# kcat/openal-soft

Measured on NVIDIA H100. Metric: voice-samples/s mixed (HRTF, bsinc24, 1024-frame updates), higher is better.
Workload: dtype f32

## Files before the change

### openal-soft_b200/csrc/mixer_kernels.cuh

```cuda
#pragma once
#include <cstddef>
#include <cstdint>
#include <cuda_runtime.h>

#include "voice_structs.hpp"
#include "async_ptx.cuh"

namespace b200mix {

constexpr int kLine = 1024;
constexpr int kHrirLen = 128;
constexpr int kHist = 64;
constexpr int kEdge = 24;
constexpr int kPad = 48;
constexpr int kResBuf = kLine + 256 + kPad;
constexpr int kSrcSizeMax = kResBuf - kEdge;
constexpr int kAccumLen = kLine + kHrirLen;
constexpr float kSilence = 0.00001f;
constexpr float kEps = 1.1920929e-07f;

constexpr uint32_t kVfStatic = 1u<<2, kVfLooping = 1u<<3, kVfHrtf = 1u<<4;
constexpr uint32_t kVfFading = 1u<<8, kVfHaveBuffer = 1u<<9, kVfCoefDirty = 1u<<10;
constexpr uint32_t kUpNoBuffer = 1u<<11;
constexpr uint32_t kVfChannelMask = 0xffu<<16;

struct alignas(16) BufferRec {
    const void *data;
    uint32_t frames, type, channels, pad;
};

struct alignas(16) VoiceRec {
    uint32_t state;
    uint32_t flags;
    uint32_t buffer, resampler;
    int32_t  pos; uint32_t frac, step, loop_start;
    uint32_t loop_end; float bsinc_sf; uint32_t bsinc_m, bsinc_l;
    uint32_t bsinc_off, tgt_delay0, tgt_delay1; float tgt_gain;
    uint32_t old_delay0, old_delay1; float old_gain; uint32_t send_mask;
    uint32_t send_slot[kMaxSends]; uint32_t pad2[2];
    float prev[kPad];
    float hist[kHist];
};

struct VoiceResult { int32_t position; uint32_t position_frac, flags, buffers_done; };

struct alignas(16) FilterRec {
    float cur[2][5]; float tgt[2][5];
    float z[2][2];
    int32_t counter[2];
    uint32_t active;
    uint32_t pad[5];
};
static_assert(sizeof(FilterRec) == 128, "FilterRec layout");

struct MixParams {
    VoiceRec *voices; const BufferRec *buffers;
    float2 *hrtf_tgt; float2 *hrtf_old;
    float *dry_cur; float *dry_tgt;
    float *partial;
    VoiceResult *results;
    const float *bsinc_tab[3];
    const float *cubic_tab[2];
    uint32_t max_voices, frames, ir_pad, cd, num_sends;
    float *xscratch;
    uint32_t *sendinfo;
    const uint32_t *order;
    uint32_t num_order;
    FilterRec *filt;
    uint32_t filt_paths;
    const float *dline;
    uint4 *qhdr; const uint32_t *queue;
    uint32_t *claim;
    const BufferRec *cbplan;
};

constexpr uint32_t kMaxQueue = 32, kNoLoop = 0xffffffffu;

constexpr uint32_t kSiSend = 1u, kSiPlaying = 2u, kSiDeferred = 4u, kSiDirty = 8u, kSiDry = 16u,
    kSiHrtf = 32u;

__device__ __forceinline__ void group_sync(int id, int count)
{
    if(id == 1) asm volatile("bar.sync 1, %0;" :: "r"(count) : "memory");
    else asm volatile("bar.sync 2, %0;" :: "r"(count) : "memory");
}

__device__ __forceinline__ bool group_sync_and(int id, int count, bool pred)
{
    uint32_t all;
    if(id == 1)
        asm volatile("{ .reg .pred p, q; setp.ne.u32 p, %1, 0; bar.red.and.pred q, 1, %2, p; selp.u32 %0, 1, 0, q; }"
            : "=r"(all) : "r"(uint32_t(pred)), "r"(count) : "memory");
    else
        asm volatile("{ .reg .pred p, q; setp.ne.u32 p, %1, 0; bar.red.and.pred q, 2, %2, p; selp.u32 %0, 1, 0, q; }"
            : "=r"(all) : "r"(uint32_t(pred)), "r"(count) : "memory");
    return all != 0u;
}

__device__ __forceinline__ bool exact16(float v)
{
    const float s = v*32768.0f;
    return s == rintf(s) && s >= -32768.0f && s <= 32767.0f;
}

__device__ __forceinline__ void prefetch_l2(const void *p)
{ asm volatile("prefetch.global.L2 [%0];" :: "l"(p)); }

__device__ __forceinline__ uint32_t sample_bytes(uint32_t type)
{ return type == 1u ? 2u : ((type == 0u || type >= 5u) ? 1u : (type == 4u ? 8u : 4u)); }

__device__ __forceinline__ void prefetch_span(const char *base, size_t bytes, size_t off,
    size_t len, int t, int gs)
{
    if(off >= bytes) return;
    if(off + len > bytes) len = bytes - off;
    const size_t first = off & ~size_t(127);
    for(size_t a = first + size_t(t)*128u;a < off + len;a += size_t(gs)*128u)
        prefetch_l2(base + a);
}

__device__ __forceinline__ float load_sample(const BufferRec &b, size_t idx)
{
    switch(b.type)
    {
    case 0: return (float(static_cast<const uint8_t*>(b.data)[idx]) - 128.0f) * (1.0f/128.0f);
    case 1: return float(static_cast<const int16_t*>(b.data)[idx]) * (1.0f/32768.0f);
    case 2: return float(static_cast<const int32_t*>(b.data)[idx]) * (1.0f/2147483648.0f);
    case 3: return static_cast<const float*>(b.data)[idx];
    case 4: return float(static_cast<const double*>(b.data)[idx]);
    }
    return 0.0f;
}

__device__ __forceinline__ void calc_buffer_size(uint32_t fracPos, uint32_t increment,
    uint32_t dstRemaining, uint32_t &dst, uint32_t &src)
{
    const uint32_t ext = increment <= 65536u;
    const uint64_t srcSize64 = ((uint64_t(dstRemaining - ext)*increment + fracPos) >> 16)
        + ext + kEdge;
    if(srcSize64 <= uint64_t(kSrcSizeMax)) { dst = dstRemaining; src = uint32_t(srcSize64); return; }
    const uint64_t dstSize64 = ((uint64_t(kSrcSizeMax - kEdge)<<16) - fracPos) / increment;
    if(dstSize64 < dstRemaining) { dst = uint32_t(dstSize64) & ~3u; src = kSrcSizeMax; return; }
    dst = dstRemaining; src = kSrcSizeMax;
}

__device__ __forceinline__ int32_t add_sat(int32_t a, int32_t b)
{
    long long r = (long long)a + b;
    r = r > 2147483647ll ? 2147483647ll : (r < -2147483648ll ? -2147483648ll : r);
    return int32_t(r);
}

__device__ __forceinline__ float to_float(uint8_t v) { return (float(v) - 128.0f) * (1.0f/128.0f); }
__device__ __forceinline__ float to_float(int16_t v) { return float(v) * (1.0f/32768.0f); }
__device__ __forceinline__ float to_float(int32_t v) { return float(v) * (1.0f/2147483648.0f); }
__device__ __forceinline__ float to_float(float v) { return v; }
__device__ __forceinline__ float to_float(double v) { return float(v); }
struct MulawByte { uint8_t v; };
struct AlawByte { uint8_t v; };
__device__ __forceinline__ float to_float(MulawByte b)
{
    const uint32_t u = (~uint32_t(b.v)) & 0xffu;
    const int s = int((((u & 0x0fu)<<3) + 0x84u) << ((u>>4)&7u)) - 0x84;
    return float((u & 0x80u) ? -s : s) * (1.0f/32768.0f);
}
__device__ __forceinline__ float to_float(AlawByte b)
{
    const uint32_t a = uint32_t(b.v) ^ 0x55u;
    const uint32_t e = (a>>4)&7u, m = a & 0x0fu;
    const int s = (e == 0u) ? int((m<<4) + 8u) : int(((m<<4) + 0x108u) << (e-1u));
    return float((a & 0x80u) ? s : -s) * (1.0f/32768.0f);
}

template<typename T> __device__ __forceinline__ T ld_raw(const T *p) { return __ldg(p); }
template<> __device__ __forceinline__ MulawByte ld_raw(const MulawByte *p)
{ return MulawByte{__ldg(reinterpret_cast<const uint8_t*>(p))}; }
template<> __device__ __forceinline__ AlawByte ld_raw(const AlawByte *p)
{ return AlawByte{__ldg(reinterpret_cast<const uint8_t*>(p))}; }

constexpr int kPackB = 688;
static_assert(kPackB >= (kResBuf + 8 + 1)/2 && kPackB + (kResBuf + 8 + 1)/2 <= kResBuf + 8 + 24
    && (kPackB % 32) == 16, "16-bit window copies must fit the float window's storage");

__device__ __forceinline__ float win_at(const float *win, bool packed, uint32_t k)
{
    if(!packed) return win[k];
    const uint16_t y = reinterpret_cast<const uint16_t*>(win)[k];
    return float(int(y) - 32768) * (1.0f/32768.0f);
}

struct FillArgs {
    float *dst; uint32_t count, uintPos, q0, firstRun, loopStart, loopSize, lastFrame, channels;
    bool looping, pastEnd, simpleWrap;
};

__device__ __forceinline__ void filter_clear(FilterRec &fr, int t)
{
    if(t < 10) fr.cur[t/5][t%5] = fr.tgt[t/5][t%5];
    else if(t < 14) fr.z[(t-10)>>1][(t-10)&1] = 0.0f;
    else if(t < 16) fr.counter[t-14] = 0;
}

template<typename T, int GS>
__device__ __forceinline__ void fill_window(const FillArgs &A, const T *__restrict__ src, int t)
{
    for(uint32_t k0 = t;k0 < A.count;k0 += 8u*GS)
    {
        T raw[8];
        #pragma unroll
        for(int u = 0;u < 8;++u)
        {
            uint32_t k = k0 + uint32_t(u)*GS;
            k = k < A.count ? k : A.count-1u;
            uint32_t q;
            if(!A.looping) q = min(A.uintPos + k, A.lastFrame);
            else if(k < A.firstRun) q = A.q0 + k;
            else if(A.simpleWrap) q = A.loopStart + (k - A.firstRun);
            else q = A.loopStart + (k - A.firstRun)%A.loopSize;
            raw[u] = ld_raw(src + size_t(q)*A.channels);
        }
        #pragma unroll
        for(int u = 0;u < 8;++u)
        {
            const uint32_t k = k0 + uint32_t(u)*GS;
            if(k < A.count) A.dst[k] = A.pastEnd ? 0.0f : to_float(raw[u]);
        }
    }
}

constexpr int kWinFloats = kResBuf + 8 + 24;
template<int CDR>
struct alignas(16) GroupSmem {
    static constexpr int kTabStride = kPad + 2;
    float win[kWinFloats];
    alignas(8) float tabF[32*kTabStride];
    alignas(8) float tabD[32*kTabStride];
    float x[CDR > 0 ? kLine : 1];
    float newGain[32];
    uint64_t tmaBar;
    uint32_t claimed;
};

struct alignas(16) FirStage {
    float x[kHist + kLine];
    float2 coefT[kHrirLen], coefO[kHrirLen];
};
static_assert(offsetof(VoiceRec, hist) % 16 == 0 && sizeof(VoiceRec) % 16 == 0,
    "VoiceRec::hist is a bulk-copy source: 16-byte aligned");

template<int GS, int OPT, int FP>
struct alignas(16) FirSmem {
    static constexpr int kLLen = FP + OPT*GS;
    static constexpr int kOLen = FP + kHist + FP + 32;
    float2 lLR[kLLen];
    float2 oLR[kOLen];
    FirStage st[2];
    uint64_t bar[2];
};

__device__ __forceinline__ float2 fma2_rn(float2 a, float2 b, float2 c)
{ return make_float2(__fmaf_rn(a.x, b.x, c.x), __fmaf_rn(a.y, b.y, c.y)); }

template<int OPT, int FP>
__device__ __forceinline__ void fir_pass(float2 (&acc)[OPT], const float2 *__restrict__ in,
    const float2 *__restrict__ coef, int irpad, int t0)
{
    constexpr int JB = 8;
    constexpr int W = OPT + JB - 1;
    for(int jb = 0;jb < irpad;jb += 2*JB)
    {
        const float2 *p = in + FP + t0 - jb - (JB-1);
        float2 w[W];
        #pragma unroll
        for(int k = 0;k < W;++k) w[k] = p[k];
        #pragma unroll
        for(int jj = 0;jj < JB;++jj)
        {
            const float2 c = coef[jb+jj];
            #pragma unroll
            for(int r = 0;r < OPT;++r)
                acc[r] = fma2_rn(c, w[r - jj + (JB-1)], acc[r]);
        }
        if(jb + JB >= irpad) break;
        #pragma unroll
        for(int k = W-1;k >= JB;--k) w[k] = w[k-JB];
        #pragma unroll
        for(int k = 0;k < JB;++k) w[k] = p[k - JB];
        #pragma unroll
        for(int jj = 0;jj < JB;++jj)
        {
            const float2 c = coef[jb+JB+jj];
            #pragma unroll
            for(int r = 0;r < OPT;++r)
                acc[r] = fma2_rn(c, w[r - jj + (JB-1)], acc[r]);
        }
    }
}

__device__ __forceinline__ uint32_t claim_voice(const MixParams &P, uint32_t &slot, int t, int bar,
    int gs, uint32_t groups)
{
    group_sync(bar, gs);
    if(t == 0)
    {
        uint32_t oi = atomicAdd(P.claim, 1u);
        if(oi >= P.num_order && atomicAdd(P.claim + 1, 1u) == groups - 1u)
        {
            atomicExch(P.claim, 0u);
            atomicExch(P.claim + 1, 0u);
        }
        slot = oi;
    }
    group_sync(bar, gs);
    return slot;
}


__device__ __forceinline__ bool voice_early_out(const MixParams &P, VoiceRec &rec, uint32_t v,
    uint32_t vstate, uint4 h1, int t)
{
    if(vstate != 1u && vstate != 2u)
    {
        if(t == 0)
        {
            if(P.results) P.results[v] = VoiceResult{int32_t(h1.x), h1.y, 1u<<7, 0u};
            if(P.sendinfo) P.sendinfo[v] = 0u;
        }
        return true;
    }
    if(h1.z < 1u)
    {
        if(t == 0)
        {
            if(vstate == 2u) rec.state = 0u;
            if(P.sendinfo) P.sendinfo[v] = 0u;
            if(P.results)
                P.results[v] = VoiceResult{int32_t(h1.x), h1.y, (vstate == 2u) ? (1u<<7) : 1u, 0u};
        }
        return true;
    }
    return false;
}

template<int GS>
__device__ __forceinline__ void build_phase_table(const MixParams &P, float *tabF, float *tabD,
    uint32_t resampler, uint32_t increment, uint4 h2, uint4 h3, int t,
    uint32_t &m, uint32_t &tapOff, uint32_t &ms)
{
    m = 0; tapOff = 0; ms = 5;
    if(resampler >= 4u)
    {
        m = h2.z;
        tapOff = kEdge - h2.w;
        const float *tab = P.bsinc_tab[(resampler-4u)>>1] + h3.x;
        const bool full = (increment > 65536u) && (resampler & 1u);
        const float sf = __uint_as_float(h2.y);
        const uint32_t rowLen = 2u*m;
        const float *tab2 = tab + 64u*m;
        ms = m + 1u;
        for(uint32_t c = t;c < rowLen;c += GS)
        {
            float *dstc = (c < m) ? (tabF + c) : (tabD + (c - m));
            #pragma unroll 1
            for(uint32_t p0 = 0;p0 < 32u;p0 += 8u)
            {
                float a[8], b[8];
                #pragma unroll
                for(int u = 0;u < 8;++u)
                {
                    a[u] = __ldg(tab + (p0+u)*rowLen + c);
                    b[u] = full ? __ldg(tab2 + (p0+u)*rowLen + c) : 0.0f;
                }
                #pragma unroll
                for(int u = 0;u < 8;++u)
                    dstc[(p0+u)*ms] = full ? fmaf(sf, b[u], a[u]) : a[u];
            }
        }
    }
    else if(resampler >= 2u)
    {
        m = 4; tapOff = kEdge - 1; ms = 5;
        const float *tab = P.cubic_tab[resampler-2u];
        for(uint32_t e = t;e < 128u;e += GS)
        {
            const uint32_t pi = e>>2, j = e&3u;
            tabF[pi*ms + j] = tab[pi*8u + j];
            tabD[pi*ms + j] = tab[pi*8u + 4u + j];
        }
    }
}

template<int GS>
__device__ __forceinline__ void prefetch_next_voices(const MixParams &P, uint32_t oi, uint32_t groups,
    int t)
{
    const uint32_t o2 = oi + 2u*groups, o1 = oi + groups;
    const uint32_t v2 = o2 < P.num_order ? P.order[o2] : 0xffffffffu;
    const uint32_t v1 = o1 < P.num_order ? P.order[o1] : 0xffffffffu;
    if(v2 < P.max_voices && t < 5)
        prefetch_l2(reinterpret_cast<const char*>(&P.voices[v2]) + t*128);
    if(v1 < P.max_voices)
    {
        const VoiceRec &nx = P.voices[v1];
        if((nx.state == 1u || nx.state == 2u) && (nx.flags & kVfHaveBuffer) && nx.step >= 1u)
        {
            const BufferRec nb = P.buffers[nx.buffer];
            const size_t fb = size_t(sample_bytes(nb.type))*nb.channels;
            const size_t bytes = size_t(nb.frames)*fb;
            const uint32_t p0 = nx.pos < 0 ? 0u : uint32_t(nx.pos);
            const size_t need = size_t((uint64_t(P.frames)*nx.step + nx.frac) >> 16) + kPad;
            const char *base = static_cast<const char*>(nb.data);
            prefetch_span(base, bytes, size_t(p0)*fb, need*fb, t, GS);
            if((nx.flags & kVfLooping) && p0 + need > nx.loop_end && nx.loop_end > p0)
                prefetch_span(base, bytes, size_t(nx.loop_start)*fb,
                    (p0 + need - nx.loop_end)*fb, t, GS);
        }
    }
}

template<int GS>
__device__ __forceinline__ void hold_end_sample(float *srcBuffer, uint32_t srcn, int t, int bar)
{
    const uint32_t avail = srcn < uint32_t(kEdge) ? srcn : uint32_t(kEdge);
    const uint32_t tofill = srcn > uint32_t(kEdge) ? srcn : uint32_t(kEdge);
    uint32_t best = 0;
    for(uint32_t i = 1;i < avail;++i)
        if(fabsf(srcBuffer[i]) < fabsf(srcBuffer[best])) best = i;
    const float held = srcBuffer[best];
    group_sync(bar, GS);
    for(uint32_t k = best+1+t;k < tofill;k += GS) srcBuffer[k] = held;
}

template<int GS>
__device__ __forceinline__ void pack_span16(float *win, const unsigned char *raw, uint32_t lead,
    uint32_t srcDelay, uint32_t count, int t, int bar)
{
    constexpr int NW = (kResBuf + 8 + 1)/2;
    constexpr int PER = (NW + GS - 1)/GS;
    static_assert((GS/32)*(32*PER - 1) >= NW + 1, "the warps' runs must cover every word");
    const uint32_t lane = uint32_t(t) & 31u;
    const uint32_t w0 = uint32_t(t >> 5)*(32u*PER - 1u) + lane;
    const uint32_t lo = uint32_t(kEdge) + srcDelay;
    const uint32_t nw = (min(lo + count + 8u, uint32_t(kResBuf + 8)) + 1u)/2u;
    const uint32_t off = lo - lead;
    const uint32_t *rw = reinterpret_cast<const uint32_t*>(raw) - int((off + 1u) >> 1);
    const uint32_t sh = (off & 1u)*16u;
    uint32_t wa[PER];
    #pragma unroll
    for(int u = 0;u < PER;++u)
    {
        const uint32_t w = w0 + uint32_t(u)*32u;
        wa[u] = (w <= nw && 2u*w + 1u >= lo) ? rw[w] : 0u;
    }
    #pragma unroll
    for(int u = 0;u < PER;++u)
    {
        const uint32_t w = w0 + uint32_t(u)*32u;
        uint32_t r1 = __shfl_sync(0xffffffffu, (u + 1 < PER && lane == 0u) ? wa[u + 1 < PER ? u + 1 : u] : wa[u],
            (lane + 1u) & 31u);
        if(u + 1 == PER && lane == 31u && w <= nw && 2u*w + 3u >= lo) r1 = rw[w + 1u];
        uint32_t a = __funnelshift_r(wa[u], r1, sh) ^ 0x80008000u;
        const int d = int(lo) - int(2u*w);
        const uint32_t m = (d >= 1 ? 0x0000ffffu : 0u) | (d >= 2 ? 0xffff0000u : 0u);
        a = (a & ~m) | (0x80008000u & m);
        if(u == 0 && w < uint32_t(kEdge/2))
            a = uint32_t(uint16_t(__float2int_rn(win[2u*w]*32768.0f) + 32768))
                | (uint32_t(uint16_t(__float2int_rn(win[2u*w + 1u]*32768.0f) + 32768)) << 16);
        wa[u] = a;
    }
    group_sync(bar, GS);
    uint32_t *pa = reinterpret_cast<uint32_t*>(win);
    uint32_t *pb = pa + kPackB;
    #pragma unroll
    for(int u = 0;u < PER;++u)
    {
        const uint32_t w = w0 + uint32_t(u)*32u;
        const uint32_t next = __shfl_sync(0xffffffffu, (u + 1 < PER && lane == 0u) ? wa[u + 1 < PER ? u + 1 : u] : wa[u],
            (lane + 1u) & 31u);
        if(w < nw)
        {
            if(u > 0 || lane > 0u || t < 32) pa[w] = wa[u];
            if(u + 1 < PER || lane < 31u) pb[w] = __funnelshift_r(wa[u], next, 16u);
        }
    }
}

template<int GS>
__device__ __forceinline__ bool stage_span_tma(float *win, uint64_t *tmaBar, uint32_t &tmaPhase,
    const BufferRec &buf, uint32_t flags, bool isQueue, bool looping, uint32_t loopStart,
    uint32_t loopEnd, uint32_t uintPos, uint32_t srcDelay, uint32_t count, bool pack, bool &packed,
    int t, int bar)
{
    if(isQueue || buf.type != 1u || buf.channels != 1u || ((flags >> 16) & 0xffu) != 0u || count == 0u)
        return false;
    const uint32_t loopSize = looping ? (loopEnd - loopStart) : 1u;
    const uint32_t q0 = !looping ? uintPos : ((uintPos < loopEnd) ? uintPos
        : ((uintPos-loopStart)%loopSize + loopStart));
    const uint32_t run1 = looping ? min(count, loopEnd - q0) : count;
    const uint32_t run2 = count - run1;
    const bool fits = looping ? (run2 <= loopSize && loopEnd <= buf.frames)
                              : (uintPos + count <= buf.frames);
    if(!fits) return false;
    const int16_t *base = static_cast<const int16_t*>(buf.data);
    const uintptr_t a1 = reinterpret_cast<uintptr_t>(base + q0);
    const uintptr_t a2 = reinterpret_cast<uintptr_t>(base + loopStart);
    const uint32_t lead1 = uint32_t(a1 & 15u) >> 1, lead2 = uint32_t(a2 & 15u) >> 1;
    const uint32_t bytes1 = ((run1 + lead1)*2u + 15u) & ~15u;
    const uint32_t bytes2 = run2 ? (((run2 + lead2)*2u + 15u) & ~15u) : 0u;
    constexpr uint32_t kWinBytes = uint32_t(kWinFloats*sizeof(float));
    unsigned char *wbytes = reinterpret_cast<unsigned char*>(win);
    unsigned char *raw2 = wbytes + kWinBytes - bytes2;
    unsigned char *raw1 = raw2 - bytes1;
    if(t == 0)
    {
        fence_proxy_async_smem();
        mbar_expect_tx(tmaBar, bytes1 + bytes2);
        bulk_g2s(raw1, reinterpret_cast<const void*>(a1 & ~uintptr_t(15)), bytes1, tmaBar);
        if(run2)
            bulk_g2s(raw2, reinterpret_cast<const void*>(a2 & ~uintptr_t(15)), bytes2, tmaBar);
    }
    mbar_wait(tmaBar, tmaPhase);
    tmaPhase ^= 1u;
    if(pack && !run2)
    {
        pack_span16<GS>(win, raw1, lead1, srcDelay, count, t, bar);
        packed = true;
        return true;
    }
    float *dst = win + kEdge + srcDelay;
    const int16_t *r1 = reinterpret_cast<const int16_t*>(raw1) + lead1;
    const int16_t *r2 = reinterpret_cast<const int16_t*>(raw2) + lead2;
    constexpr int PERW = (kSrcSizeMax + GS - 1)/GS;
    float v[PERW];
    #pragma unroll
    for(int u = 0;u < PERW;++u)
    {
        const uint32_t k = uint32_t(t) + uint32_t(u)*GS;
        int16_t x = 0;
        if(k < count) x = k < run1 ? r1[k] : r2[k - run1];
        v[u] = to_float(x);
    }
    group_sync(bar, GS);
    #pragma unroll
    for(int u = 0;u < PERW;++u)
    {
        const uint32_t k = uint32_t(t) + uint32_t(u)*GS;
        if(k < count) dst[k] = v[u];
    }
    return true;
}

template<int GS>
__device__ __forceinline__ bool gather_span(const MixParams &P, const BufferRec &buf, uint32_t flags,
    bool isQueue, uint4 qh, const uint32_t *qitems, bool looping, uint32_t loopStart, uint32_t loopEnd,
    uint32_t uintPos, uint32_t count, float *dst, int t, int bar)
{
    uint32_t done = 0, item = qh.x ? qh.y : kNoLoop, qpos = uintPos;
    bool more = true, winInt = true;
    while(more)
    {
        BufferRec rb = buf;
        FillArgs fa;
        if(!isQueue)
        {
            const uint32_t loopSize = looping ? (loopEnd - loopStart) : 1u;
            const uint32_t q0 = !looping ? uintPos : ((uintPos < loopEnd) ? uintPos
                : ((uintPos-loopStart)%loopSize + loopStart));
            const uint32_t firstRun = looping ? (loopEnd - q0) : 0u;
            const uint32_t lastFrame = buf.frames ? buf.frames-1u : 0u;
            const bool pastEnd = !looping && !(buf.frames > uintPos);
            const bool simpleWrap = looping && count <= firstRun + loopSize;
            fa = FillArgs{dst, count, uintPos, q0, firstRun, loopStart, loopSize,
                lastFrame, buf.channels, looping, pastEnd, simpleWrap};
            done = count; more = false;
        }
        else
        {
            bool found = false;
            while(item != kNoLoop && done < count)
            {
                rb = P.buffers[qitems[item]];
                if(qpos >= rb.frames)
                {
                    qpos -= rb.frames;
                    item = (item + 1u < qh.x) ? item + 1u : qh.z;
                    continue;
                }
                found = true;
                break;
            }
            if(!found) break;
            const uint32_t run = min(count - done, rb.frames - qpos);
            fa = FillArgs{dst + done, run, qpos, qpos, 0u, 0u, 1u, rb.frames-1u,
                rb.channels, false, false, false};
            done += run; qpos = 0u;
            item = (item + 1u < qh.x) ? item + 1u : qh.z;
            more = done < count;
        }
        winInt = winInt && (rb.type <= 1u || rb.type >= 5u);
        const uint32_t ch = ((flags >> 16) & 0xffu) < rb.channels ? ((flags >> 16) & 0xffu) : 0u;
        switch(rb.type)
        {
        case 0: fill_window<uint8_t, GS>(fa, static_cast<const uint8_t*>(rb.data) + ch, t); break;
        case 1: fill_window<int16_t, GS>(fa, static_cast<const int16_t*>(rb.data) + ch, t); break;
        case 2: fill_window<int32_t, GS>(fa, static_cast<const int32_t*>(rb.data) + ch, t); break;
        case 3: fill_window<float, GS>(fa, static_cast<const float*>(rb.data) + ch, t); break;
        case 4: fill_window<double, GS>(fa, static_cast<const double*>(rb.data) + ch, t); break;
        case 5: fill_window<MulawByte, GS>(fa, static_cast<const MulawByte*>(rb.data) + ch, t); break;
        default: fill_window<AlawByte, GS>(fa, static_cast<const AlawByte*>(rb.data) + ch, t); break;
        }
    }
    if(done < count)
    {
        group_sync(bar, GS);
        const float held = done ? dst[done-1u] : 0.0f;
        for(uint32_t k = done + t;k < count;k += GS) dst[k] = held;
    }
    return winInt;
}

template<int GS>
__device__ __forceinline__ void pack_window16(float *win, uint32_t srcn, int t, int bar)
{
    constexpr int PER = (kResBuf + 8 + GS - 1)/GS;
    const uint32_t L = min(uint32_t(kEdge) + srcn + 8u, uint32_t(kResBuf + 8));
    float v[PER];
    #pragma unroll
    for(int u = 0;u < PER;++u)
    {
        const uint32_t k = uint32_t(t) + uint32_t(u)*GS;
        v[u] = k < L ? win[k] : 0.0f;
    }
    group_sync(bar, GS);
    uint16_t *pa = reinterpret_cast<uint16_t*>(win);
    uint16_t *pb = pa + 2*kPackB;
    #pragma unroll
    for(int u = 0;u < PER;++u)
    {
        const uint32_t k = uint32_t(t) + uint32_t(u)*GS;
        if(k < L)
        {
            const uint16_t y = uint16_t(__float2int_rn(v[u]*32768.0f) + 32768);
            pa[k] = y;
            if(k) pb[k-1u] = y;
        }
    }
    group_sync(bar, GS);
}

template<int GS>
__device__ __forceinline__ void resample_chunk(const float *win, const float *tabF, const float *tabD,
    float *xs, uint32_t loaded, uint32_t dstn, uint32_t increment, uint32_t fracPos,
    uint32_t resampler, uint32_t m, uint32_t tapOff, uint32_t ms, bool packedWin, int t)
{
    const float *srcBuffer = win + kEdge;
    if(increment == 65536u && fracPos == 0u)
    {
        for(uint32_t k = t;k < dstn;k += GS) xs[loaded+k] = srcBuffer[k];
    }
    else if(packedWin)
    {
        const uint32_t *wordsA = reinterpret_cast<const uint32_t*>(win);
        const uint32_t *wordsB = wordsA + kPackB;
        const float2 bias = make_float2(-8421376.0f, -8421376.0f);
        const float2 one = make_float2(1.0f, 1.0f);
        for(uint32_t k = t;k < dstn;k += 2u*GS)
        {
            const uint32_t kB = k + GS;
            const bool hasB = kB < dstn;
            const uint64_t fpA = uint64_t(k)*increment + fracPos;
            const uint64_t fpB = uint64_t(hasB ? kB : k)*increment + fracPos;
            const uint32_t fracA = uint32_t(fpA) & 0xffffu, fracB = uint32_t(fpB) & 0xffffu;
            const float pfA = float(fracA & 2047u) * (1.0f/2048.0f);
            const float pfB = float(fracB & 2047u) * (1.0f/2048.0f);
            const float *FA = tabF + (fracA>>11)*ms, *DA = tabD + (fracA>>11)*ms;
            const float *FB = tabF + (fracB>>11)*ms, *DB = tabD + (fracB>>11)*ms;
            const uint32_t posA = tapOff + uint32_t(fpA>>16), posB = tapOff + uint32_t(fpB>>16);
            const uint32_t *wA = ((posA & 1u) ? wordsB : wordsA) + (posA >> 1);
            const uint32_t *wB = ((posB & 1u) ? wordsB : wordsA) + (posB >> 1);
            const float2 pA = make_float2(pfA, pfA), pB = make_float2(pfB, pfB);
            float2 a0 = make_float2(0.0f, 0.0f), a1 = a0, b0 = a0, b1 = a0;
            for(uint32_t j = 0;j < m;j += 4)
            {
                const uint32_t wa0 = wA[(j>>1)], wa1 = wA[(j>>1)+1u];
                const uint32_t wb0 = wB[(j>>1)], wb1 = wB[(j>>1)+1u];
                const float2 sA0 = fma2_rn(make_float2(__uint_as_float(__byte_perm(wa0, 0x4B00u, 0x5410u)),
                    __uint_as_float(__byte_perm(wa0, 0x4B00u, 0x5432u))), one, bias);
                const float2 sA1 = fma2_rn(make_float2(__uint_as_float(__byte_perm(wa1, 0x4B00u, 0x5410u)),
                    __uint_as_float(__byte_perm(wa1, 0x4B00u, 0x5432u))), one, bias);
                const float2 sB0 = fma2_rn(make_float2(__uint_as_float(__byte_perm(wb0, 0x4B00u, 0x5410u)),
                    __uint_as_float(__byte_perm(wb0, 0x4B00u, 0x5432u))), one, bias);
                const float2 sB1 = fma2_rn(make_float2(__uint_as_float(__byte_perm(wb1, 0x4B00u, 0x5410u)),
                    __uint_as_float(__byte_perm(wb1, 0x4B00u, 0x5432u))), one, bias);
                const float2 cA0 = fma2_rn(pA, make_float2(DA[j+0], DA[j+1]), make_float2(FA[j+0], FA[j+1]));
                const float2 cB0 = fma2_rn(pB, make_float2(DB[j+0], DB[j+1]), make_float2(FB[j+0], FB[j+1]));
                const float2 cA1 = fma2_rn(pA, make_float2(DA[j+2], DA[j+3]), make_float2(FA[j+2], FA[j+3]));
                const float2 cB1 = fma2_rn(pB, make_float2(DB[j+2], DB[j+3]), make_float2(FB[j+2], FB[j+3]));
                a0 = fma2_rn(cA0, sA0, a0);
                b0 = fma2_rn(cB0, sB0, b0);
                a1 = fma2_rn(cA1, sA1, a1);
                b1 = fma2_rn(cB1, sB1, b1);
            }
            xs[loaded+k] = ((a0.x + a1.x) + (a0.y + a1.y)) * (1.0f/32768.0f);
            if(hasB) xs[loaded+kB] = ((b0.x + b1.x) + (b0.y + b1.y)) * (1.0f/32768.0f);
        }
    }
    else if(resampler >= 2u)
    {
        const float *vals = win + tapOff;
        for(uint32_t k = t;k < dstn;k += 2u*GS)
        {
            const uint32_t kB = k + GS;
            const bool hasB = kB < dstn;
            const uint64_t fpA = uint64_t(k)*increment + fracPos;
            const uint64_t fpB = uint64_t(hasB ? kB : k)*increment + fracPos;
            const uint32_t fracA = uint32_t(fpA) & 0xffffu, fracB = uint32_t(fpB) & 0xffffu;
            const float pfA = float(fracA & 2047u) * (1.0f/2048.0f);
            const float pfB = float(fracB & 2047u) * (1.0f/2048.0f);
            const float *FA = tabF + (fracA>>11)*ms, *DA = tabD + (fracA>>11)*ms;
            const float *FB = tabF + (fracB>>11)*ms, *DB = tabD + (fracB>>11)*ms;
            const float *svA = vals + uint32_t(fpA>>16), *svB = vals + uint32_t(fpB>>16);
            const float2 pA = make_float2(pfA, pfA), pB = make_float2(pfB, pfB);
            float2 a0 = make_float2(0.0f, 0.0f), a1 = a0, b0 = a0, b1 = a0;
            for(uint32_t j = 0;j < m;j += 4)
            {
                const float2 cA0 = fma2_rn(pA, make_float2(DA[j+0], DA[j+1]), make_float2(FA[j+0], FA[j+1]));
                const float2 cB0 = fma2_rn(pB, make_float2(DB[j+0], DB[j+1]), make_float2(FB[j+0], FB[j+1]));
                const float2 cA1 = fma2_rn(pA, make_float2(DA[j+2], DA[j+3]), make_float2(FA[j+2], FA[j+3]));
                const float2 cB1 = fma2_rn(pB, make_float2(DB[j+2], DB[j+3]), make_float2(FB[j+2], FB[j+3]));
                a0 = fma2_rn(cA0, make_float2(svA[j+0], svA[j+1]), a0);
                b0 = fma2_rn(cB0, make_float2(svB[j+0], svB[j+1]), b0);
                a1 = fma2_rn(cA1, make_float2(svA[j+2], svA[j+3]), a1);
                b1 = fma2_rn(cB1, make_float2(svB[j+2], svB[j+3]), b1);
            }
            xs[loaded+k] = (a0.x + a1.x) + (a0.y + a1.y);
            if(hasB) xs[loaded+kB] = (b0.x + b1.x) + (b0.y + b1.y);
        }
    }
    else
    {
        const float *vals = srcBuffer;
        for(uint32_t k = t;k < dstn;k += GS)
        {
            const uint64_t fp = uint64_t(k)*increment + fracPos;
            const uint32_t pos = uint32_t(fp>>16), frac = uint32_t(fp) & 0xffffu;
            if(resampler == 0u) xs[loaded+k] = vals[pos];
            else
            {
                const float a = vals[pos], b = vals[pos+1];
                xs[loaded+k] = a + (b-a)*(float(frac)*(1.0f/65536.0f));
            }
        }
    }
}

template<int GS>
__device__ __forceinline__ void advance_chunk(float *win, float *prev, bool packedWin, bool silent,
    bool playing, uint32_t n, uint32_t &loaded, uint32_t dstn, uint32_t increment, uint32_t &fracPos,
    int32_t &intPos, int t, int bar)
{
    const uint32_t loadEnd = loaded + dstn;
    if(!silent && playing && n > loaded && n <= loadEnd)
    {
        const uint32_t dstOffset = n - loaded;
        const uint32_t srcOffset = uint32_t((uint64_t(dstOffset)*increment + fracPos) >> 16);
        for(int k = t;k < kPad;k += GS) prev[k] = win_at(win, packedWin, srcOffset + uint32_t(k));
    }
    loaded = loadEnd;
    if(loaded < n)
    {
        fracPos += dstn*increment;
        const uint32_t srcOffset = fracPos >> 16;
        fracPos &= 0xffffu;
        if(silent) intPos = add_sat(intPos, int32_t(srcOffset));
        else
        {
            if(intPos < 0) intPos += int32_t(srcOffset);
            else intPos = add_sat(intPos, int32_t(srcOffset));
            float carry = 0.0f;
            if(t < kPad) carry = win_at(win, packedWin, srcOffset + uint32_t(t));
            float carry2 = 0.0f;
            if(GS < kPad && t + GS < kPad) carry2 = win_at(win, packedWin, srcOffset + uint32_t(t) + GS);
            group_sync(bar, GS);
            if(t < kPad) win[t] = carry;
            if(GS < kPad && t + GS < kPad) win[t + GS] = carry2;
        }
    }
}

template<int GS, int CDR>
__device__ __forceinline__ void park_voice(const MixParams &P, const float *xs, uint32_t v,
    uint32_t sendMask, bool defer, bool isHrtf, bool playing, bool dirty, uint32_t counter, int t)
{
    const uint32_t n = P.frames;
    const bool sends = P.num_sends && sendMask;
    const bool park = sends || defer || CDR == 0;
    if(CDR > 0 && park)
        for(uint32_t k = t;k < n;k += GS) P.xscratch[size_t(v)*kLine + k] = xs[k];
    if(t == 0)
// ... 47 lines not shown
__device__ __forceinline__ void write_back_voice(const MixParams &P, VoiceRec &rec, uint32_t v,
    uint4 h1, uint32_t flags, uint32_t vstate, uint32_t increment, bool haveBuffer, bool isQueue,
    uint4 qh, const uint32_t *qitems, bool looping, uint32_t loopStart, uint32_t loopEnd,
    uint32_t bufFrames)
{
    uint32_t newFlags = (flags | kVfFading) & ~kVfCoefDirty;
    uint32_t newState = vstate;
    uint32_t buffersDone = 0u;
    int32_t pos = int32_t(h1.x); uint32_t frac = h1.y;
    if(vstate == 2u) newState = 0u;
    else
    {
        frac += increment*P.frames;
        const uint32_t done = frac >> 16;
        pos = add_sat(pos, int32_t(done));
        frac &= 0xffffu;
        if(haveBuffer && pos > 0 && isQueue)
        {
            uint32_t item = qh.x ? qh.y : kNoLoop;
            while(item != kNoLoop)
            {
                const uint32_t len = P.buffers[qitems[item]].frames;
                if(len > uint32_t(pos)) break;
                pos -= int32_t(len);
                ++buffersDone;
                item = (item + 1u < qh.x) ? item + 1u : qh.z;
            }
            if(item == kNoLoop) { newFlags &= ~kVfHaveBuffer; newState = 2u; }
            else if(item != qh.y) P.qhdr[v].y = item;
        }
        else if(haveBuffer && pos > 0)
        {
            if(looping)
            {
                uint32_t up = uint32_t(pos);
                if(up >= loopEnd)
                    pos = int32_t((up-loopStart)%(loopEnd-loopStart) + loopStart);
            }
            else if(uint32_t(pos) >= bufFrames)
            {
                newFlags &= ~kVfHaveBuffer;
                newState = 2u;
            }
        }
        if(!haveBuffer) newState = 2u;
        rec.pos = pos; rec.frac = frac;
    }
    rec.flags = newFlags;
    rec.state = newState;
    if(P.results)
        P.results[v] = VoiceResult{pos, frac,
            newState == 1u ? 1u : (newState == 2u ? 2u : (1u<<7)), buffersDone};
}

template<int GS, int GROUPS, int CDR>
__device__ __forceinline__ void store_partial_row(const float (&accD)[CDR][kLine/GS], unsigned char *smem,
    float *partial, int g, int t)
{
    constexpr int SPT = kLine / GS;
    const size_t row = blockIdx.x;
    __syncthreads();
    float *stage = reinterpret_cast<float*>(smem);
    float *pd = partial + row*(size_t(CDR)*kLine);
    if(GROUPS == 1)
    {
        #pragma unroll
        for(int c = 0;c < CDR;++c)
            #pragma unroll
            for(int r = 0;r < SPT;++r)
                pd[c*kLine + t + r*GS] = accD[c][r];
    }
    else
    {
        for(int gg = 0;gg < GROUPS;++gg)
        {
            if(g == gg)
            {
                #pragma unroll
                for(int c = 0;c < CDR;++c)
                    #pragma unroll
                    for(int r = 0;r < SPT;++r)
                    {
                        float *dst = stage + c*kLine + t + r*GS;
                        if(gg == 0) *dst = accD[c][r]; else *dst += accD[c][r];
                    }
            }
            __syncthreads();
        }
        for(int o = threadIdx.x;o < CDR*kLine;o += GS*GROUPS) pd[o] = stage[o];
    }
}

constexpr int kMixGS = 64, kMixGroups = 2;

template<int GS, int GROUPS, int CDR>
__global__ void __launch_bounds__(GS*GROUPS, GS*GROUPS != 128 ? 1 : (CDR == 0 ? 5 : 3))
k_mix_voices(const MixParams P)
{
    using Smem = GroupSmem<CDR>;
    static_assert(CDR == 0 || sizeof(Smem)*GROUPS >= size_t(CDR)*kLine*sizeof(float),
        "the partial row is staged in the groups' storage");
    extern __shared__ __align__(16) unsigned char smem_raw[];
    const int g = threadIdx.x / GS;
    const int t = threadIdx.x % GS;
    Smem &S = reinterpret_cast<Smem*>(smem_raw)[g];
    const int bar = 1 + g;
    constexpr int SPT = kLine / GS;

    float accD[CDR > 0 ? CDR : 1][SPT];
    #pragma unroll
    for(int c = 0;c < (CDR > 0 ? CDR : 1);++c)
        #pragma unroll
        for(int r = 0;r < SPT;++r) accD[c][r] = 0.0f;

    const uint32_t n = P.frames;
    if(t == 0) { mbar_init(&S.tmaBar, 1u); mbar_fence_init(); }
    uint32_t tmaPhase = 0u;
    group_sync(bar, GS);

    const uint32_t groups = gridDim.x*GROUPS;
    for(uint32_t oi = CDR > 0 ? blockIdx.x*GROUPS + g : claim_voice(P, S.claimed, t, bar, GS, groups);
        oi < P.num_order;
        oi = CDR > 0 ? oi + groups : claim_voice(P, S.claimed, t, bar, GS, groups))
    {
        const uint32_t v = P.order[oi];
        VoiceRec &rec = P.voices[v];
        const uint4 *hp = reinterpret_cast<const uint4*>(&rec);
        const uint4 h0 = hp[0], h1 = hp[1], h2 = hp[2], h3 = hp[3];
        const uint32_t vstate = h0.x;
        if(voice_early_out(P, rec, v, vstate, h1, t)) continue;
        const uint32_t increment = h1.z;
        const uint32_t flags = h0.y;
        const bool haveBuffer = (flags & kVfHaveBuffer) != 0;
        const BufferRec rb = P.buffers[haveBuffer ? h0.z : 0u];
        const BufferRec buf = (haveBuffer && rb.pad && P.cbplan) ? P.cbplan[rb.pad - 1u] : rb;
        const uint32_t cbSlot = haveBuffer ? buf.pad : 0u;
        const uint32_t loopStart = h1.w, loopEnd = h2.x;
        int32_t intPos = int32_t(h1.x);
        uint32_t fracPos = h1.y;
        bool looping = (flags & kVfLooping) != 0 && cbSlot == 0u;
        if((flags & kVfStatic) && looping && haveBuffer && intPos >= 0
            && uint32_t(intPos) >= loopEnd)
            looping = false;
        const uint32_t resampler = h0.w;
        const bool isQueue = !(flags & kVfStatic) && P.qhdr != nullptr && cbSlot == 0u;
        const uint4 qh = isQueue ? P.qhdr[v] : make_uint4(0u, 0u, kNoLoop, 0u);
        const uint32_t *qitems = P.queue + size_t(v)*kMaxQueue;
        const bool isHrtf = CDR == 0 && P.ir_pad != 0u && (flags & kVfHrtf);
        const bool dirty = (flags & kVfCoefDirty) != 0;
        FilterRec *dfilt = P.filt ? P.filt + size_t(v)*P.filt_paths : nullptr;
        const bool defer = dfilt && dfilt->active;
        const bool playing = vstate == 1u;

        for(int k = t;k < kPad;k += GS) S.win[k] = rec.prev[k];
        uint32_t m, tapOff, ms;
        build_phase_table<GS>(P, S.tabF, S.tabD, resampler, increment, h2, h3, t, m, tapOff, ms);
        float *xs = CDR > 0 ? S.x : P.xscratch + size_t(v)*kLine;
        if(CDR == 0) prefetch_next_voices<GS>(P, oi, groups, t);

        for(uint32_t loaded = 0;loaded < n;)
        {
            uint32_t dstn, srcn;
            calc_buffer_size(fracPos, increment, n-loaded, dstn, srcn);
            uint32_t srcDelay = 0;
            bool silent = false;
            bool packedWin = false;
            if(dstn == 0u) { dstn = n - loaded; silent = true; }
            if(intPos < 0)
            {
                srcDelay = uint32_t(-intPos);
                if(srcDelay >= srcn) silent = true;
            }
            const bool histExact = group_sync_and(bar, GS, t >= kEdge || exact16(S.win[t]));
            if(silent)
            {
                for(uint32_t k = t;k < dstn;k += GS) xs[loaded+k] = 0.0f;
                for(uint32_t k = t;k < srcn;k += GS) S.win[kEdge+k] = 0.0f;
            }
            else
            {
                float *srcBuffer = S.win + kEdge;
                bool winInt = false;
                const bool pack = resampler >= 4u && !(increment == 65536u && fracPos == 0u) && histExact;
                if(!haveBuffer) hold_end_sample<GS>(srcBuffer, srcn, t, bar);
                else
                {
                    const uint32_t uintPos = intPos < 0 ? 0u : uint32_t(intPos);
                    const uint32_t count = srcn - srcDelay;
                    for(uint32_t k = t;k < srcDelay;k += GS) srcBuffer[k] = 0.0f;
                    winInt = stage_span_tma<GS>(S.win, &S.tmaBar, tmaPhase, buf, flags, isQueue, looping,
                            loopStart, loopEnd, uintPos, srcDelay, count, pack, packedWin, t, bar)
                        || gather_span<GS>(P, buf, flags, isQueue, qh, qitems, looping, loopStart, loopEnd,
                            uintPos, count, srcBuffer + srcDelay, t, bar);
                }
                group_sync(bar, GS);

                if(pack && winInt && !packedWin)
                {
                    pack_window16<GS>(S.win, srcn, t, bar);
                    packedWin = true;
                }
                resample_chunk<GS>(S.win, S.tabF, S.tabD, xs, loaded, dstn, increment, fracPos,
                    resampler, m, tapOff, ms, packedWin, t);
            }
            advance_chunk<GS>(S.win, rec.prev, packedWin, silent, playing, n, loaded, dstn, increment,
                fracPos, intPos, t, bar);
        }
        group_sync(bar, GS);

        const uint32_t counter = (flags & kVfFading) ? (n < 64u ? n : 64u) : 0u;
        if(P.sendinfo)
            park_voice<GS, CDR>(P, xs, v, rec.send_mask, defer, isHrtf, playing, dirty, counter, t);
        if(dfilt && !defer) filter_clear(*dfilt, t);
        if constexpr(CDR > 0)
            if(!defer)
                mix_dry<GS, CDR>(accD, xs, S.newGain, P.dry_cur + size_t(v)*P.cd, P.dry_tgt + size_t(v)*P.cd,
                    P.cd, n, counter, playing, t);
        if(t == 0)
            write_back_voice(P, rec, v, h1, flags, vstate, increment, haveBuffer, isQueue, qh, qitems,
                looping, loopStart, loopEnd, buf.frames);
        group_sync(bar, GS);
        if(CDR > 0 && !defer) store_dry_gains(P.dry_cur + size_t(v)*P.cd, S.newGain, P.cd, t);
        group_sync(bar, GS);
    }

    if constexpr(CDR > 0) store_partial_row<GS, GROUPS, CDR>(accD, smem_raw, P.partial, g, t);
}

template<int GROUPS, int CDR>
union DeferredSmem {
    struct { float x[kLine]; float newGain[32]; } group[GROUPS];
    float stage[CDR*kLine];
};

template<int GS, int GROUPS, int CDR>
__global__ void __launch_bounds__(GS*GROUPS)
k_mix_deferred(const MixParams P)
{
    extern __shared__ __align__(16) unsigned char smem_raw[];
    const int g = threadIdx.x / GS;
    const int t = threadIdx.x % GS;
    auto &S = reinterpret_cast<DeferredSmem<GROUPS, CDR>*>(smem_raw)->group[g];
    const int bar = 1 + g;
    constexpr int SPT = kLine / GS;

    float accD[CDR][SPT];
    #pragma unroll
    for(int c = 0;c < CDR;++c)
        #pragma unroll
        for(int r = 0;r < SPT;++r) accD[c][r] = 0.0f;

    const uint32_t n = P.frames;
    const uint32_t groups = gridDim.x*GROUPS;
    for(uint32_t oi = blockIdx.x*GROUPS + g;oi < P.num_order;oi += groups)
    {
        const uint32_t v = P.order[oi];
        const uint32_t info = P.sendinfo[v];
        if(!(info & kSiDeferred)) continue;
        const float *fl = P.dline + size_t(v)*kLine;
        for(uint32_t k = t;k < n;k += GS) S.x[k] = fl[k];
        group_sync(bar, GS);
        mix_dry<GS, CDR>(accD, S.x, S.newGain, P.dry_cur + size_t(v)*P.cd, P.dry_tgt + size_t(v)*P.cd,
            P.cd, n, (info >> 8) & 0xffu, (info & kSiPlaying) != 0, t);
        group_sync(bar, GS);
        store_dry_gains(P.dry_cur + size_t(v)*P.cd, S.newGain, P.cd, t);
    }

    store_partial_row<GS, GROUPS, CDR>(accD, smem_raw, P.partial, g, t);
}

constexpr int kFirGS = 64, kFirGroups = 2, kFirCtasPerSm = 4;

__device__ __forceinline__ uint32_t next_hrtf_voice(const MixParams &P, uint32_t oi, uint32_t stride,
    uint32_t &v, uint32_t &info)
{
    for(;oi < P.num_order;oi += stride)
    {
        v = P.order[oi];
        info = P.sendinfo[v];
        if(info & kSiHrtf) break;
    }
    return oi;
}

__device__ __forceinline__ void fir_stage_issue(const MixParams &P, FirStage &B, uint64_t *bar,
    uint32_t v, uint32_t info, uint32_t n)
{
    const uint32_t lineBytes = (n & ~3u)*4u, irBytes = P.ir_pad*8u;
    const bool dirty = (info & kSiDirty) != 0;
    const float *line = ((info & kSiDeferred) ? P.dline : P.xscratch) + size_t(v)*kLine;
    fence_proxy_async_smem();
    mbar_expect_tx(bar, kHist*4u + lineBytes + (dirty ? 2u : 1u)*irBytes);
    bulk_g2s(B.x, P.voices[v].hist, kHist*4u, bar);
    if(lineBytes) bulk_g2s(B.x + kHist, line, lineBytes, bar);
    bulk_g2s(B.coefT, P.hrtf_tgt + size_t(v)*P.ir_pad, irBytes, bar);
    if(dirty) bulk_g2s(B.coefO, P.hrtf_old + size_t(v)*P.ir_pad, irBytes, bar);
}

template<int OPT, int FP>
__global__ void __launch_bounds__(kFirGS*kFirGroups, kFirCtasPerSm)
k_hrtf_fir(const MixParams P)
{
    constexpr int GS = kFirGS, GROUPS = kFirGroups;
    using Smem = FirSmem<GS, OPT, FP>;
    extern __shared__ __align__(16) unsigned char smem_raw[];
    const int g = threadIdx.x / GS;
    const int t = threadIdx.x % GS;
    Smem &S = reinterpret_cast<Smem*>(smem_raw)[g];
    const int bar = 1 + g;
    const int t0 = OPT*t;
    const uint32_t n = P.frames;

    float2 acc[OPT];
    #pragma unroll
    for(int r = 0;r < OPT;++r) acc[r] = make_float2(0.0f, 0.0f);

    for(int i = t;i < FP;i += GS) S.lLR[i] = make_float2(0.0f, 0.0f);
    for(int i = FP + int(n) + t;i < Smem::kLLen;i += GS) S.lLR[i] = make_float2(0.0f, 0.0f);
    if(t == 0) { mbar_init(&S.bar[0], 1u); mbar_init(&S.bar[1], 1u); mbar_fence_init(); }
    group_sync(bar, GS);

    const uint32_t stride = gridDim.x*GROUPS;
    uint32_t v = 0u, info = 0u;
    uint32_t oi = next_hrtf_voice(P, blockIdx.x*GROUPS + g, stride, v, info);
    if(t == 0 && oi < P.num_order) fir_stage_issue(P, S.st[0], &S.bar[0], v, info, n);
    uint32_t parity = 0u;
    for(int b = 0;oi < P.num_order;b ^= 1)
    {
        VoiceRec &rec = P.voices[v];
        const uint4 *hp = reinterpret_cast<const uint4*>(&rec);
        const uint4 h3 = hp[3], h4 = hp[4];

        uint32_t vN = 0u, infoN = 0u;
        const uint32_t oiN = next_hrtf_voice(P, oi + stride, stride, vN, infoN);
        if(t == 0 && oiN < P.num_order) fir_stage_issue(P, S.st[b^1], &S.bar[b^1], vN, infoN, n);

        FirStage &B = S.st[b];
        const bool playing = (info & kSiPlaying) != 0;
        const bool dirty = (info & kSiDirty) != 0;
        const uint32_t counter = (info >> 8) & 0xffu;

        const float *line = ((info & kSiDeferred) ? P.dline : P.xscratch) + size_t(v)*kLine;
        for(uint32_t k = (n & ~3u) + t;k < n;k += GS) B.x[kHist + k] = line[k];
        mbar_wait(&S.bar[b], (parity >> b) & 1u);
        parity ^= 1u << b;
        if(n & 3u) group_sync(bar, GS);
// ... 1250 lines not shown
```

Before: 30.77 billion.

## Widen resampler source window so a full update fits in one chunk

Adds a wider source-window capacity (about two update lengths) that is used when the voice's whole span can be read directly from a non-queued buffer. Most voices then resample an update in one chunk instead of several, which removes repeated staging, packing and group syncs. The packing and conversion loops are rewritten as strided loops, replacing the fixed per-thread register arrays that were sized to the old window. Shared memory per group grows, which may lower occupancy.

```diff
diff --git a/openal-soft_b200/csrc/mixer_kernels.cuh b/openal-soft_b200/csrc/mixer_kernels.cuh
--- a/openal-soft_b200/csrc/mixer_kernels.cuh
+++ b/openal-soft_b200/csrc/mixer_kernels.cuh
@@ -15,6 +15,8 @@
 constexpr int kPad = 48;
 constexpr int kResBuf = kLine + 256 + kPad;
 constexpr int kSrcSizeMax = kResBuf - kEdge;
+constexpr int kSrcSizeWide = 2*kLine + kEdge;
+constexpr int kWinLen = kEdge + kSrcSizeWide;
 constexpr int kAccumLen = kLine + kHrirLen;
 constexpr float kSilence = 0.00001f;
 constexpr float kEps = 1.1920929e-07f;
@@ -132,16 +134,31 @@
     return 0.0f;
 }
 
+__device__ __forceinline__ uint64_t span_size(uint32_t fracPos, uint32_t increment, uint32_t dstRemaining)
+{
+    const uint32_t ext = increment <= 65536u;
+    return ((uint64_t(dstRemaining - ext)*increment + fracPos) >> 16) + ext + kEdge;
+}
+
 __device__ __forceinline__ void calc_buffer_size(uint32_t fracPos, uint32_t increment,
-    uint32_t dstRemaining, uint32_t &dst, uint32_t &src)
-{
-    const uint32_t ext = increment <= 65536u;
-    const uint64_t srcSize64 = ((uint64_t(dstRemaining - ext)*increment + fracPos) >> 16)
-        + ext + kEdge;
-    if(srcSize64 <= uint64_t(kSrcSizeMax)) { dst = dstRemaining; src = uint32_t(srcSize64); return; }
-    const uint64_t dstSize64 = ((uint64_t(kSrcSizeMax - kEdge)<<16) - fracPos) / increment;
-    if(dstSize64 < dstRemaining) { dst = uint32_t(dstSize64) & ~3u; src = kSrcSizeMax; return; }
-    dst = dstRemaining; src = kSrcSizeMax;
+    uint32_t dstRemaining, uint32_t srcCap, uint32_t &dst, uint32_t &src)
+{
+    const uint64_t srcSize64 = span_size(fracPos, increment, dstRemaining);
+    if(srcSize64 <= uint64_t(srcCap)) { dst = dstRemaining; src = uint32_t(srcSize64); return; }
+    const uint64_t dstSize64 = ((uint64_t(srcCap - kEdge)<<16) - fracPos) / increment;
+    if(dstSize64 < dstRemaining) { dst = uint32_t(dstSize64) & ~3u; src = srcCap; return; }
+    dst = dstRemaining; src = srcCap;
+}
+
+__device__ __forceinline__ bool span_runs(const BufferRec &buf, bool looping, uint32_t loopStart,
+    uint32_t loopEnd, uint32_t uintPos, uint32_t count, uint32_t &q0, uint32_t &run1)
+{
+    const uint32_t loopSize = looping ? (loopEnd - loopStart) : 1u;
+    q0 = !looping ? uintPos : ((uintPos < loopEnd) ? uintPos
+        : ((uintPos-loopStart)%loopSize + loopStart));
+    run1 = looping ? min(count, loopEnd - q0) : count;
+    return looping ? (count - run1 <= loopSize && loopEnd <= buf.frames)
+                   : (uint64_t(uintPos) + count <= buf.frames);
 }
 
 __device__ __forceinline__ int32_t add_sat(int32_t a, int32_t b)
@@ -178,9 +195,13 @@
 template<> __device__ __forceinline__ AlawByte ld_raw(const AlawByte *p)
 { return AlawByte{__ldg(reinterpret_cast<const uint8_t*>(p))}; }
 
-constexpr int kPackB = 688;
-static_assert(kPackB >= (kResBuf + 8 + 1)/2 && kPackB + (kResBuf + 8 + 1)/2 <= kResBuf + 8 + 24
+constexpr int kWinFloats = kWinLen + 8 + 24;
+constexpr int kPackWords = (kWinLen + 8 + 1)/2;
+constexpr int kPackB = 1072;
+static_assert(kPackB >= kPackWords + 1 && kPackB + kPackWords <= kWinFloats
     && (kPackB % 32) == 16, "16-bit window copies must fit the float window's storage");
+static_assert(2*(kEdge + 2*kSrcSizeWide + 9) + 4 + 28 <= 4*kWinFloats && 4*kWinLen + 60 <= 4*kWinFloats,
+    "a window copy must not reach the raw span's bytes of later positions");
 
 __device__ __forceinline__ float win_at(const float *win, bool packed, uint32_t k)
 {
@@ -228,7 +249,6 @@
     }
 }
 
-constexpr int kWinFloats = kResBuf + 8 + 24;
 template<int CDR>
 struct alignas(16) GroupSmem {
     static constexpr int kTabStride = kPad + 2;
@@ -431,58 +451,45 @@
     for(uint32_t k = best+1+t;k < tofill;k += GS) srcBuffer[k] = held;
 }
 
+__device__ __forceinline__ uint32_t pack2_16(float v0, float v1)
+{
+    return uint32_t(uint16_t(__float2int_rn(v0*32768.0f) + 32768))
+        | (uint32_t(uint16_t(__float2int_rn(v1*32768.0f) + 32768)) << 16);
+}
+
+template<int GS>
+__device__ __forceinline__ void pack_copy_b(float *win, uint32_t nw, int t)
+{
+    const uint32_t *pa = reinterpret_cast<const uint32_t*>(win);
+    uint32_t *pb = reinterpret_cast<uint32_t*>(win) + kPackB;
+    for(uint32_t w = t;w < nw;w += GS) pb[w] = __funnelshift_r(pa[w], pa[w + 1u], 16u);
+}
+
 template<int GS>
 __device__ __forceinline__ void pack_span16(float *win, const unsigned char *raw, uint32_t lead,
     uint32_t srcDelay, uint32_t count, int t, int bar)
 {
-    constexpr int NW = (kResBuf + 8 + 1)/2;
-    constexpr int PER = (NW + GS - 1)/GS;
-    static_assert((GS/32)*(32*PER - 1) >= NW + 1, "the warps' runs must cover every word");
-    const uint32_t lane = uint32_t(t) & 31u;
-    const uint32_t w0 = uint32_t(t >> 5)*(32u*PER - 1u) + lane;
+    static_assert(kEdge <= 32, "warp 0 stores the history's words and the ones over its floats");
     const uint32_t lo = uint32_t(kEdge) + srcDelay;
-    const uint32_t nw = (min(lo + count + 8u, uint32_t(kResBuf + 8)) + 1u)/2u;
+    const uint32_t nw = (lo + count + 8u + 1u)/2u;
     const uint32_t off = lo - lead;
     const uint32_t *rw = reinterpret_cast<const uint32_t*>(raw) - int((off + 1u) >> 1);
     const uint32_t sh = (off & 1u)*16u;
-    uint32_t wa[PER];
-    #pragma unroll
-    for(int u = 0;u < PER;++u)
-    {
-        const uint32_t w = w0 + uint32_t(u)*32u;
-        wa[u] = (w <= nw && 2u*w + 1u >= lo) ? rw[w] : 0u;
-    }
-    #pragma unroll
-    for(int u = 0;u < PER;++u)
-    {
-        const uint32_t w = w0 + uint32_t(u)*32u;
-        uint32_t r1 = __shfl_sync(0xffffffffu, (u + 1 < PER && lane == 0u) ? wa[u + 1 < PER ? u + 1 : u] : wa[u],
-            (lane + 1u) & 31u);
-        if(u + 1 == PER && lane == 31u && w <= nw && 2u*w + 3u >= lo) r1 = rw[w + 1u];
-        uint32_t a = __funnelshift_r(wa[u], r1, sh) ^ 0x80008000u;
+    uint32_t *pa = reinterpret_cast<uint32_t*>(win);
+    const uint32_t hist = t < kEdge/2 ? pack2_16(win[2*t], win[2*t + 1]) : 0u;
+    __syncwarp();
+    for(uint32_t w = t;w < nw;w += GS)
+    {
+        const uint32_t r0 = 2u*w + 1u >= lo ? rw[w] : 0u;
+        const uint32_t r1 = 2u*w + 3u >= lo ? rw[w + 1u] : 0u;
+        uint32_t a = __funnelshift_r(r0, r1, sh) ^ 0x80008000u;
         const int d = int(lo) - int(2u*w);
         const uint32_t m = (d >= 1 ? 0x0000ffffu : 0u) | (d >= 2 ? 0xffff0000u : 0u);
         a = (a & ~m) | (0x80008000u & m);
-        if(u == 0 && w < uint32_t(kEdge/2))
-            a = uint32_t(uint16_t(__float2int_rn(win[2u*w]*32768.0f) + 32768))
-                | (uint32_t(uint16_t(__float2int_rn(win[2u*w + 1u]*32768.0f) + 32768)) << 16);
-        wa[u] = a;
+        pa[w] = w < uint32_t(kEdge/2) ? hist : a;
     }
     group_sync(bar, GS);
-    uint32_t *pa = reinterpret_cast<uint32_t*>(win);
-    uint32_t *pb = pa + kPackB;
-    #pragma unroll
-    for(int u = 0;u < PER;++u)
-    {
-        const uint32_t w = w0 + uint32_t(u)*32u;
-        const uint32_t next = __shfl_sync(0xffffffffu, (u + 1 < PER && lane == 0u) ? wa[u + 1 < PER ? u + 1 : u] : wa[u],
-            (lane + 1u) & 31u);
-        if(w < nw)
-        {
-            if(u > 0 || lane > 0u || t < 32) pa[w] = wa[u];
-            if(u + 1 < PER || lane < 31u) pb[w] = __funnelshift_r(wa[u], next, 16u);
-        }
-    }
+    pack_copy_b<GS>(win, nw, t);
 }
 
 template<int GS>
@@ -493,14 +500,9 @@
 {
     if(isQueue || buf.type != 1u || buf.channels != 1u || ((flags >> 16) & 0xffu) != 0u || count == 0u)
         return false;
-    const uint32_t loopSize = looping ? (loopEnd - loopStart) : 1u;
-    const uint32_t q0 = !looping ? uintPos : ((uintPos < loopEnd) ? uintPos
-        : ((uintPos-loopStart)%loopSize + loopStart));
-    const uint32_t run1 = looping ? min(count, loopEnd - q0) : count;
+    uint32_t q0, run1;
+    if(!span_runs(buf, looping, loopStart, loopEnd, uintPos, count, q0, run1)) return false;
     const uint32_t run2 = count - run1;
-    const bool fits = looping ? (run2 <= loopSize && loopEnd <= buf.frames)
-                              : (uintPos + count <= buf.frames);
-    if(!fits) return false;
     const int16_t *base = static_cast<const int16_t*>(buf.data);
     const uintptr_t a1 = reinterpret_cast<uintptr_t>(base + q0);
     const uintptr_t a2 = reinterpret_cast<uintptr_t>(base + loopStart);
@@ -527,25 +529,29 @@
         packed = true;
         return true;
     }
+    for(uint32_t k = t;k < srcDelay;k += GS) win[kEdge + k] = 0.0f;
     float *dst = win + kEdge + srcDelay;
     const int16_t *r1 = reinterpret_cast<const int16_t*>(raw1) + lead1;
     const int16_t *r2 = reinterpret_cast<const int16_t*>(raw2) + lead2;
-    constexpr int PERW = (kSrcSizeMax + GS - 1)/GS;
-    float v[PERW];
-    #pragma unroll
-    for(int u = 0;u < PERW;++u)
-    {
-        const uint32_t k = uint32_t(t) + uint32_t(u)*GS;
-        int16_t x = 0;
-        if(k < count) x = k < run1 ? r1[k] : r2[k - run1];
-        v[u] = to_float(x);
-    }
-    group_sync(bar, GS);
-    #pragma unroll
-    for(int u = 0;u < PERW;++u)
-    {
-        const uint32_t k = uint32_t(t) + uint32_t(u)*GS;
-        if(k < count) dst[k] = v[u];
+    constexpr int U = 8;
+    for(uint32_t k0 = 0;k0 < count;k0 += U*GS)
+    {
+        float v[U];
+        #pragma unroll
+        for(int u = 0;u < U;++u)
+        {
+            const uint32_t k = k0 + uint32_t(t) + uint32_t(u)*GS;
+            int16_t x = 0;
+            if(k < count) x = k < run1 ? r1[k] : r2[k - run1];
+            v[u] = to_float(x);
+        }
+        group_sync(bar, GS);
+        #pragma unroll
+        for(int u = 0;u < U;++u)
+        {
+            const uint32_t k = k0 + uint32_t(t) + uint32_t(u)*GS;
+            if(k < count) dst[k] = v[u];
+        }
     }
     return true;
 }
@@ -622,29 +628,28 @@
 template<int GS>
 __device__ __forceinline__ void pack_window16(float *win, uint32_t srcn, int t, int bar)
 {
-    constexpr int PER = (kResBuf + 8 + GS - 1)/GS;
-    const uint32_t L = min(uint32_t(kEdge) + srcn + 8u, uint32_t(kResBuf + 8));
-    float v[PER];
-    #pragma unroll
-    for(int u = 0;u < PER;++u)
-    {
-        const uint32_t k = uint32_t(t) + uint32_t(u)*GS;
-        v[u] = k < L ? win[k] : 0.0f;
+    const uint32_t L = min(uint32_t(kEdge) + srcn + 8u, uint32_t(kWinLen + 8));
+    constexpr int U = 8;
+    uint16_t *pa = reinterpret_cast<uint16_t*>(win);
+    for(uint32_t k0 = 0;k0 < L;k0 += U*GS)
+    {
+        float v[U];
+        #pragma unroll
+        for(int u = 0;u < U;++u)
+        {
+            const uint32_t k = k0 + uint32_t(t) + uint32_t(u)*GS;
+            v[u] = k < L ? win[k] : 0.0f;
+        }
+        group_sync(bar, GS);
+        #pragma unroll
+        for(int u = 0;u < U;++u)
+        {
+            const uint32_t k = k0 + uint32_t(t) + uint32_t(u)*GS;
+            if(k < L) pa[k] = uint16_t(__float2int_rn(v[u]*32768.0f) + 32768);
+        }
     }
     group_sync(bar, GS);
-    uint16_t *pa = reinterpret_cast<uint16_t*>(win);
-    uint16_t *pb = pa + 2*kPackB;
-    #pragma unroll
-    for(int u = 0;u < PER;++u)
-    {
-        const uint32_t k = uint32_t(t) + uint32_t(u)*GS;
-        if(k < L)
-        {
-            const uint16_t y = uint16_t(__float2int_rn(v[u]*32768.0f) + 32768);
-            pa[k] = y;
-            if(k) pb[k-1u] = y;
-        }
-    }
+    pack_copy_b<GS>(win, (L + 1u)/2u, t);
     group_sync(bar, GS);
 }
 
@@ -998,6 +1003,15 @@
         const bool defer = dfilt && dfilt->active;
         const bool playing = vstate == 1u;
 
+        uint32_t srcCap = kSrcSizeMax;
+        {
+            const uint64_t span = span_size(fracPos, increment, n);
+            uint32_t q0, run1;
+            if(haveBuffer && !isQueue && intPos >= 0 && span <= 0xffffffffu
+                && span_runs(buf, looping, loopStart, loopEnd, uint32_t(intPos), uint32_t(span), q0, run1))
+                srcCap = kSrcSizeWide;
+        }
+
         for(int k = t;k < kPad;k += GS) S.win[k] = rec.prev[k];
         uint32_t m, tapOff, ms;
         build_phase_table<GS>(P, S.tabF, S.tabD, resampler, increment, h2, h3, t, m, tapOff, ms);
@@ -1007,7 +1021,7 @@
         for(uint32_t loaded = 0;loaded < n;)
         {
             uint32_t dstn, srcn;
-            calc_buffer_size(fracPos, increment, n-loaded, dstn, srcn);
+            calc_buffer_size(fracPos, increment, n-loaded, srcCap, dstn, srcn);
             uint32_t srcDelay = 0;
             bool silent = false;
             bool packedWin = false;
@@ -1033,11 +1047,14 @@
                 {
                     const uint32_t uintPos = intPos < 0 ? 0u : uint32_t(intPos);
                     const uint32_t count = srcn - srcDelay;
-                    for(uint32_t k = t;k < srcDelay;k += GS) srcBuffer[k] = 0.0f;
                     winInt = stage_span_tma<GS>(S.win, &S.tmaBar, tmaPhase, buf, flags, isQueue, looping,
-                            loopStart, loopEnd, uintPos, srcDelay, count, pack, packedWin, t, bar)
-                        || gather_span<GS>(P, buf, flags, isQueue, qh, qitems, looping, loopStart, loopEnd,
-                            uintPos, count, srcBuffer + srcDelay, t, bar);
+                            loopStart, loopEnd, uintPos, srcDelay, count, pack, packedWin, t, bar);
+                    if(!winInt)
+                    {
+                        for(uint32_t k = t;k < srcDelay;k += GS) srcBuffer[k] = 0.0f;
+                        winInt = gather_span<GS>(P, buf, flags, isQueue, qh, qitems, looping, loopStart,
+                            loopEnd, uintPos, count, srcBuffer + srcDelay, t, bar);
+                    }
                 }
                 group_sync(bar, GS);
 
```

Measured after the change: 31.45 billion, median of 6. +2.2%, better.
